# Hansard-T/FHE-Linformer

Measured on AMD Instinct MI355X. Metric: encrypted Linformer-d128 forward ms/sample, lower is better.
Workload: dtype u64

## Files before the change

fhe-linformer_amd/csrc/kernels_elem.hip:

```cpp
#include <hip/hip_runtime.h>
#include <cstdlib>
#include <type_traits>
#include "kernels.h"
#include "kernels_elem.h"

namespace fhelin {
namespace {

typedef u64 u64x2 __attribute__((ext_vector_type(2)));

__device__ __forceinline__ Barrett load_barrett(const DeviceTables& t, int limb) {
    Barrett b;
    b.q = t.moduli[limb];
    b.r0 = t.barrett[2 * limb];
    b.r1 = t.barrett[2 * limb + 1];
    return b;
}

template <int OP>
__global__ __launch_bounds__(256) void ew_binary_kernel(DeviceTables t, u64* out, const u64* a, const u64* b, int b_mod,
                                                        int limb_first, int limb_count) {
    const int v = blockIdx.y;
    const int limb = limb_first + v % limb_count;
    const size_t n2 = (size_t)blockIdx.x * 256 + threadIdx.x;
    const size_t row = ((size_t)1 << t.log_n) >> 1;
    const u64x2 x = reinterpret_cast<const u64x2*>(a)[(size_t)v * row + n2];
    const u64x2 y = reinterpret_cast<const u64x2*>(b)[(size_t)(v % b_mod) * row + n2];
    u64x2 r;
    if (OP == 0) {
        const Barrett br = load_barrett(t, limb);
        r.x = mul_mod(x.x, y.x, br);
        r.y = mul_mod(x.y, y.y, br);
    } else if (OP == 1) {
        const u64 q = t.moduli[limb];
        r.x = add_mod(x.x, y.x, q);
        r.y = add_mod(x.y, y.y, q);
    } else {
        const u64 q = t.moduli[limb];
        r.x = sub_mod(x.x, y.x, q);
        r.y = sub_mod(x.y, y.y, q);
    }
    reinterpret_cast<u64x2*>(out)[(size_t)v * row + n2] = r;
}

template <int OP>
__global__ __launch_bounds__(256) void ew_items_kernel(DeviceTables t, EwItems it, int limb_count) {
    const int item = blockIdx.y / it.vecs, v = blockIdx.y % it.vecs;
    const int limb = v % limb_count;
    const size_t n2 = (size_t)blockIdx.x * 256 + threadIdx.x;
    const size_t row = ((size_t)1 << t.log_n) >> 1;
    const u64x2 x = reinterpret_cast<const u64x2*>(it.a[item])[(size_t)v * row + n2];
    u64x2 r = x;
    if (OP != 4 && (OP != 3 || v < it.b_vecs)) {
        const u64x2 y = reinterpret_cast<const u64x2*>(it.b[item])[(size_t)(v % it.b_vecs) * row + n2];
        if (OP == 0) {
            const Barrett br = load_barrett(t, limb);
            r.x = mul_mod(x.x, y.x, br);
            r.y = mul_mod(x.y, y.y, br);
        } else if (OP == 2) {
            const u64 q = t.moduli[limb];
            r.x = sub_mod(x.x, y.x, q);
            r.y = sub_mod(x.y, y.y, q);
        } else {
            const u64 q = t.moduli[limb];
            r.x = add_mod(x.x, y.x, q);
            r.y = add_mod(x.y, y.y, q);
        }
    }
    reinterpret_cast<u64x2*>(it.out[item])[(size_t)v * row + n2] = r;
}

__global__ __launch_bounds__(256) void ew_dot_kernel(DeviceTables t, u64* out, EwItems it, int limb_count) {
    const int v = blockIdx.y;
    const Barrett br = load_barrett(t, v % limb_count);
    const size_t n2 = (size_t)blockIdx.x * 256 + threadIdx.x;
    const size_t row = ((size_t)1 << t.log_n) >> 1;
    Acc128 ax = {0, 0}, ay = {0, 0};
    for (int i = 0; i < it.n; ++i) {
        const u64x2 x = reinterpret_cast<const u64x2*>(it.a[i])[(size_t)v * row + n2];
        const u64x2 y = reinterpret_cast<const u64x2*>(it.b[i])[(size_t)(v % it.b_vecs) * row + n2];
        acc_mac(ax, x.x, y.x);
        acc_mac(ay, x.y, y.y);
    }
    u64x2 r;
    r.x = barrett_reduce128(ax.lo, ax.hi, br);
    r.y = barrett_reduce128(ay.lo, ay.hi, br);
    reinterpret_cast<u64x2*>(out)[(size_t)v * row + n2] = r;
}

template <int NA>
__global__ __launch_bounds__(256) __attribute__((amdgpu_waves_per_eu(NA <= 8 ? 4 : 3))) void ew_dot_groups_kernel(DeviceTables t, EwDotGroups d) {
    const unsigned nx = gridDim.x, nblk = gridDim.x * gridDim.y;
    unsigned id = blockIdx.y * nx + blockIdx.x;
    if ((nblk & 7) == 0) id = (id & 7) * (nblk >> 3) + (id >> 3);
    const int comp = (int)(id & 1);
    const unsigned rest = id >> 1;
    const int xb = (int)(rest % (unsigned)d.nbatch);
    const int bx = (int)((rest / (unsigned)d.nbatch) % nx), tt = (int)((rest / (unsigned)d.nbatch) / nx);
    const Barrett br = load_barrett(t, tt);
    const size_t n2 = (size_t)bx * 256 + threadIdx.x;
    const size_t row = ((size_t)1 << t.log_n) >> 1;
    const size_t op = (size_t)tt * row + n2, oc = (size_t)(comp * d.ell + tt) * row + n2;
    u64x2 a[NA];
#pragma unroll
    for (int b = 0; b < NA; ++b) a[b] = reinterpret_cast<const u64x2*>(d.a[b] + (size_t)xb * d.a_stride[b])[oc];
    if constexpr (NA <= 8) {
        u64x2 w[NA], wn[NA];
#pragma unroll
        for (int b = 0; b < NA; ++b) w[b] = reinterpret_cast<const u64x2*>(d.p[0][b])[op];
        for (int g = 0; g < d.ng; ++g) {
            const int gn = g + 1 < d.ng ? g + 1 : g;
#pragma unroll
            for (int b = 0; b < NA; ++b) wn[b] = reinterpret_cast<const u64x2*>(d.p[gn][b])[op];
            Acc128 x = {0, 0}, y = {0, 0};
            const u32 m = d.pmask[g];
#pragma unroll
            for (int b = 0; b < NA; ++b)
                if (m >> b & 1u) {
                    acc_mac(x, a[b].x, w[b].x);
                    acc_mac(y, a[b].y, w[b].y);
                }
            u64x2 r;
            r.x = barrett_reduce128(x.lo, x.hi, br);
            r.y = barrett_reduce128(y.lo, y.hi, br);
            reinterpret_cast<u64x2*>(d.out[g] + (size_t)xb * d.out_stride[g])[oc] = r;
#pragma unroll
            for (int b = 0; b < NA; ++b) w[b] = wn[b];
        }
    } else {
        for (int g = 0; g < d.ng; ++g) {
            Acc128 x = {0, 0}, y = {0, 0};
            const u32 m = d.pmask[g];
#pragma unroll
            for (int b0 = 0; b0 < NA; b0 += 8) {
                u64x2 w[8];
#pragma unroll
                for (int b = 0; b < 8; ++b) w[b] = reinterpret_cast<const u64x2*>(d.p[g][b0 + b])[op];
#pragma unroll
                for (int b = 0; b < 8; ++b)
                    if (m >> (b0 + b) & 1u) {
                        acc_mac(x, a[b0 + b].x, w[b].x);
                        acc_mac(y, a[b0 + b].y, w[b].y);
                    }
            }
            u64x2 r;
            r.x = barrett_reduce128(x.lo, x.hi, br);
            r.y = barrett_reduce128(y.lo, y.hi, br);
            reinterpret_cast<u64x2*>(d.out[g] + (size_t)xb * d.out_stride[g])[oc] = r;
        }
    }
}

template <int SH>
__device__ __forceinline__ u64 pack_sh(u64 x) { return (x & ((1ull << SH) - 1)) | ((x >> SH) << 32); }
template <int SH>
__device__ __forceinline__ void acc_flush_sh(const Acc30& a, u64& lo, u64& hi) {
    u64 t = lo + a.s0;
    hi += (t < lo);
    lo = t;
    t = lo + (a.s1 << SH);
    hi += (a.s1 >> (64 - SH)) + (t < lo);
    lo = t;
    t = lo + (a.s2 << (2 * SH));
    hi += (a.s2 >> (64 - 2 * SH)) + (t < lo);
    lo = t;
}

#ifndef WSPLIT
#define WSPLIT 1
#endif
template <int I0, int I1, class F>
__device__ __forceinline__ void static_for(F&& f) {
    if constexpr (I0 < I1) {
        f(std::integral_constant<int, I0>{});
        static_for<I0 + 1, I1>(f);
    }
}

template <int SH>
__device__ __forceinline__ void cyclic_body(const DeviceTables& t, const EwCyclic& d, const Barrett& br, u64 (*ml)[256]) {
    constexpr int P = EwCyclic::PERIOD, G = 2;
    const int tt = blockIdx.y;
    const size_t N = (size_t)1 << t.log_n;
    const size_t n = (size_t)blockIdx.x * 256 + threadIdx.x;
    const size_t oc = (size_t)(blockIdx.z * d.ell + tt) * N + n;
    const u32 bm = (u32)(((size_t)tt * N + n) * 8), bc = (u32)(oc * 8);
    auto ld = [](const u64* p, u32 byte_off) -> u64 { return *reinterpret_cast<const u64*>(reinterpret_cast<const char*>(p) + byte_off); };
    {
        u64 mv[P];
#pragma unroll
        for (int j = 0; j < P; ++j) mv[j] = ld(d.m[j], bm);
#pragma unroll
        for (int j = 0; j < P; ++j) ml[j][threadIdx.x] = pack_sh<SH>(mv[j]);
    }
    __builtin_amdgcn_sched_barrier(0);
    u64 a[P];
#pragma unroll
    for (int i = 0; i < P; ++i) a[i] = ld(d.a[i], bc);
#pragma unroll
    for (int i = 0; i < P; ++i) a[i] = i < d.n ? pack_sh<SH>(a[i]) : 0;
#pragma unroll 1
    for (int k = 0; k < P; k += G) {
        u64 lo[G], hi[G];
        Acc30 x[G];
        static_for<0, G>([&](auto I) __attribute__((always_inline)) {
            lo[decltype(I)::value] = hi[decltype(I)::value] = 0;
            x[decltype(I)::value] = Acc30{0, 0, 0};
        });
        static_for<0, P / 8>([&](auto I0) __attribute__((always_inline)) {
            constexpr int i0 = 8 * decltype(I0)::value;
            static_for<i0, i0 + 8>([&](auto I) __attribute__((always_inline)) {
                constexpr int i = decltype(I)::value;
                const u64 w = ml[(i + k) & (P - 1)][threadIdx.x];
                const u32 w0 = (u32)w, w1 = (u32)(w >> 32);
                static_for<0, G>([&](auto Gi) __attribute__((always_inline)) {
                    constexpr int g = decltype(Gi)::value;
                    constexpr int ii = (i - g) & (P - 1);
                    mac30(x[g], (u32)a[ii], (u32)(a[ii] >> 32), w0, w1);
                });
            });
            __builtin_amdgcn_sched_barrier(0);
            if constexpr (SH == 30) {
                static_for<0, G>([&](auto Gi) __attribute__((always_inline)) {
                    constexpr int g = decltype(Gi)::value;
                    acc_flush_sh<30>(x[g], lo[g], hi[g]);
                    x[g] = Acc30{0, 0, 0};
                    if constexpr (i0 == 8) {
                        lo[g] = barrett_reduce128(lo[g], hi[g], br);
                        hi[g] = 0;
                    }
                });
            }
        });
        static_for<0, G>([&](auto Gi) __attribute__((always_inline)) {
            constexpr int g = decltype(Gi)::value;
            if constexpr (SH != 30) acc_flush_sh<SH>(x[g], lo[g], hi[g]);
            d.out[k + g][oc] = barrett_reduce128(lo[g], hi[g], br);
        });
    }
}

__global__ __launch_bounds__(256, 2) void ew_cyclic_dot_kernel(DeviceTables t, EwCyclic d) {
    __shared__ u64 ml[EwCyclic::PERIOD][256];
    const Barrett br = load_barrett(t, blockIdx.y);
    if ((br.q >> 53) == 0)
        cyclic_body<27>(t, d, br, ml);
    else
        cyclic_body<30>(t, d, br, ml);
}

template <int O0, int SH, int G>
__device__ __forceinline__ void window_segment(const EwWindow& d, const Barrett& br, const u64 (&cur)[EwWindow::W], const u64 (&prv)[EwWindow::W],
                                               const u64 (*ml)[256], size_t oc, u64 (&pre)[G]) {
    constexpr int P = EwWindow::W;
#pragma unroll 1
    for (int oo = 0; oo < 8; oo += G) {
        u64 lo[G], hi[G];
        Acc30 x[G][WSPLIT];
        static_for<0, G>([&](auto I) __attribute__((always_inline)) {
            constexpr int i = decltype(I)::value;
            lo[i] = pre[i];
            hi[i] = 0;
            static_for<0, WSPLIT>([&](auto U) __attribute__((always_inline)) { x[i][decltype(U)::value] = Acc30{0, 0, 0}; });
        });
        if (d.accumulate && O0 + oo + G < P) {
            static_for<0, G>([&](auto I) __attribute__((always_inline)) { pre[decltype(I)::value] = d.out[O0 + oo + G + decltype(I)::value][oc]; });
        }
        static_for<0, P / 8>([&](auto J0) __attribute__((always_inline)) {
            constexpr int j0 = 8 * decltype(J0)::value;
            static_for<j0, j0 + 8>([&](auto J) __attribute__((always_inline)) {
                constexpr int j = decltype(J)::value;
                constexpr int c = O0 - j;
                u64 w;
                if constexpr (c >= 0)
                    w = ml[oo + c][threadIdx.x];
                else if constexpr (c + (8 - G) < 0)
                    w = ml[oo + c + P][threadIdx.x];
                else
                    w = ml[(oo + c) & (P - 1)][threadIdx.x];
                const u32 w0 = (u32)w, w1 = (u32)(w >> 32);
                static_for<0, G>([&](auto I) __attribute__((always_inline)) {
                    constexpr int i = decltype(I)::value;
                    constexpr int jj = (j + i) & (P - 1);
                    constexpr int e = jj - O0 - i;
                    u64 a;
                    if constexpr (jj < O0 || e <= 0)
                        a = cur[jj];
                    else if constexpr (jj >= O0 + 8 || e > 8 - G)
                        a = prv[jj];
                    else
                        a = oo >= e ? cur[jj] : prv[jj];
                    mac30(x[i][j % WSPLIT], (u32)a, (u32)(a >> 32), w0, w1);
                });
            });
            if constexpr (SH == 30) {
                static_for<0, G>([&](auto I) __attribute__((always_inline)) {
                    constexpr int i = decltype(I)::value;
                    static_for<0, WSPLIT>([&](auto U) __attribute__((always_inline)) {
                        acc_flush_sh<30>(x[i][decltype(U)::value], lo[i], hi[i]);
                        x[i][decltype(U)::value] = Acc30{0, 0, 0};
                    });
                    if constexpr (j0 == 8 || j0 == 24) {
                        lo[i] = barrett_reduce128(lo[i], hi[i], br);
                        hi[i] = 0;
                    }
                });
            }
        });
        static_for<0, G>([&](auto I) __attribute__((always_inline)) {
            constexpr int i = decltype(I)::value;
            if constexpr (SH != 30) {
                static_for<0, WSPLIT>([&](auto U) __attribute__((always_inline)) { acc_flush_sh<SH>(x[i][decltype(U)::value], lo[i], hi[i]); });
                lo[i] = barrett_reduce128(lo[i], hi[i], br);
            }
            d.out[O0 + oo + i][oc] = lo[i];
        });
    }
}

template <int SH, int G>
__device__ __forceinline__ void window_body(const DeviceTables& t, const EwWindow& d, const Barrett& br, u64 (*ml)[256]) {
    constexpr int P = EwWindow::W;
    const int tt = blockIdx.y;
    const size_t N = (size_t)1 << t.log_n;
    const size_t n = (size_t)blockIdx.x * 256 + threadIdx.x;
    const size_t om = (size_t)tt * N + n, oc = (size_t)(blockIdx.z * d.ell + tt) * N + n;
    {
        u64 mv[P];
#pragma unroll
        for (int k = 0; k < P; ++k) mv[k] = d.m[k][om];
#pragma unroll
        for (int k = 0; k < P; ++k) ml[k][threadIdx.x] = pack_sh<SH>(mv[k]);
    }
    u64 cur[P], prv[P];
    auto load_cur = [&](int j0) {
#pragma unroll
        for (int j = j0; j < j0 + 8; ++j) cur[j] = d.cur[j][oc];
#pragma unroll
        for (int j = j0; j < j0 + 8; ++j) cur[j] = (d.cur_mask >> j & 1u) ? pack_sh<SH>(cur[j]) : 0;
    };
#pragma unroll
    for (int j = 0; j < P; ++j) prv[j] = d.prev[j][oc];
#pragma unroll
    for (int j = 0; j < P; ++j) prv[j] = (d.prev_mask >> j & 1u) ? pack_sh<SH>(prv[j]) : 0;
    load_cur(0);
    load_cur(8);
    u64 pre[G];
#pragma unroll
    for (int i = 0; i < G; ++i) pre[i] = d.accumulate ? d.out[i][oc] : 0;
    window_segment<0, SH, G>(d, br, cur, prv, ml, oc, pre);
    load_cur(16);
    window_segment<8, SH, G>(d, br, cur, prv, ml, oc, pre);
    load_cur(24);
    window_segment<16, SH, G>(d, br, cur, prv, ml, oc, pre);
    window_segment<24, SH, G>(d, br, cur, prv, ml, oc, pre);
}

template <int G>
__global__ __launch_bounds__(256, 2) void ew_window_dot_kernel(DeviceTables t, EwWindow d) {
    __shared__ u64 ml[EwWindow::W][256];
    const Barrett br = load_barrett(t, blockIdx.y);
    if ((br.q >> 53) == 0)
        window_body<27, G>(t, d, br, ml);
    else
        window_body<30, G>(t, d, br, ml);
}

__global__ __launch_bounds__(256) void ew_muladd_kernel(DeviceTables t, u64* out, const u64* acc, const u64* a, const u64* b,
                                                        int b_mod, int limb_first, int limb_count) {
    const int v = blockIdx.y;
    const int limb = limb_first + v % limb_count;
    const size_t n2 = (size_t)blockIdx.x * 256 + threadIdx.x;
    const size_t row = ((size_t)1 << t.log_n) >> 1;
    const Barrett br = load_barrett(t, limb);
    const u64x2 x = reinterpret_cast<const u64x2*>(a)[(size_t)v * row + n2];
    const u64x2 y = reinterpret_cast<const u64x2*>(b)[(size_t)(v % b_mod) * row + n2];
    const u64x2 c = reinterpret_cast<const u64x2*>(acc)[(size_t)v * row + n2];
    u64x2 r;
    r.x = add_mod(c.x, mul_mod(x.x, y.x, br), br.q);
    r.y = add_mod(c.y, mul_mod(x.y, y.y, br), br.q);
    reinterpret_cast<u64x2*>(out)[(size_t)v * row + n2] = r;
}

__global__ __launch_bounds__(256) void ew_neg_kernel(DeviceTables t, u64* out, const u64* a, int limb_first, int limb_count) {
    const int v = blockIdx.y;
    const u64 q = t.moduli[limb_first + v % limb_count];
    const size_t n2 = (size_t)blockIdx.x * 256 + threadIdx.x;
    const size_t row = ((size_t)1 << t.log_n) >> 1;
    const u64x2 x = reinterpret_cast<const u64x2*>(a)[(size_t)v * row + n2];
    u64x2 r;
    r.x = neg_mod(x.x, q);
    r.y = neg_mod(x.y, q);
    reinterpret_cast<u64x2*>(out)[(size_t)v * row + n2] = r;
}

__global__ __launch_bounds__(256) void ew_scalar_kernel(DeviceTables t, u64* out, const u64* a, ScalarSet sc, int limb_first,
                                                        int limb_count, int in_limbs) {
    const int v = blockIdx.y;
    const int li = v % limb_count;
    const u64 q = t.moduli[limb_first + li];
    const u64 w = sc.v[2 * li], ws = sc.v[2 * li + 1];
    const size_t n2 = (size_t)blockIdx.x * 256 + threadIdx.x;
    const size_t row = ((size_t)1 << t.log_n) >> 1;
    const size_t vin = in_limbs > 0 ? (size_t)(v / limb_count) * in_limbs + li : (size_t)v;
    const u64x2 x = reinterpret_cast<const u64x2*>(a)[vin * row + n2];
    u64x2 r;
    r.x = mul_shoup(x.x, w, ws, q);
    r.y = mul_shoup(x.y, w, ws, q);
    reinterpret_cast<u64x2*>(out)[(size_t)v * row + n2] = r;
}

__global__ __launch_bounds__(256) void ew_scalar_items_kernel(DeviceTables t, EwScalarItems d, u64* __restrict__ out,
                                                              const u64* __restrict__ consts) {
    const int vecs = d.npoly * d.ell;
    const int item = blockIdx.y / vecs, v = blockIdx.y % vecs;
    const int limb = v % d.ell;
    const u64 q = t.moduli[limb];
    const u64* k = consts + ((size_t)item * d.ell + limb) * 2;
    const u64 w = k[0], ws = k[1];
    const size_t n2 = (size_t)blockIdx.x * 256 + threadIdx.x;
    const size_t row = ((size_t)1 << t.log_n) >> 1;
    const size_t vin = (size_t)(v / d.ell) * d.in_limbs[item] + limb;
    const u64x2 x = reinterpret_cast<const u64x2*>(d.a[item])[vin * row + n2];
    u64x2 r;
    r.x = mul_shoup(x.x, w, ws, q);
    r.y = mul_shoup(x.y, w, ws, q);
    reinterpret_cast<u64x2*>(out)[((size_t)item * vecs + v) * row + n2] = r;
}

__global__ __launch_bounds__(256) void ew_scaled_diff_kernel(DeviceTables t, EwScaledDiff d, const u64* __restrict__ consts) {
    const int item = blockIdx.y / d.vecs, v = blockIdx.y % d.vecs;
    const int limb = v % d.ell;
    const u64 q = t.moduli[limb];
    const u64* k = consts + ((size_t)item * d.ell + limb) * 4;
    const u64 a = k[0], as = k[1], c = k[2], cs = k[3];
    const size_t n2 = (size_t)blockIdx.x * 256 + threadIdx.x;
    const size_t row = ((size_t)1 << t.log_n) >> 1;
    const size_t at = (size_t)v * row + n2;
    const u64x2 x = reinterpret_cast<const u64x2*>(d.u[item])[at];
    const u64x2 y = reinterpret_cast<const u64x2*>(d.w[item])[at];
    u64x2 r;
    r.x = sub_mod(mul_shoup(x.x, a, as, q), mul_shoup(y.x, c, cs, q), q);
    r.y = sub_mod(mul_shoup(x.y, a, as, q), mul_shoup(y.y, c, cs, q), q);
    reinterpret_cast<u64x2*>(d.out[item])[at] = r;
}

__global__ __launch_bounds__(256) void ew_addscalar_kernel(DeviceTables t, u64* out, const u64* a, ScalarSet sc, int limb_first,
                                                           int limb_count, int add_vecs) {
    const int v = blockIdx.y;
    const int li = v % limb_count;
    const u64 q = t.moduli[limb_first + li];
    const u64 w = v < add_vecs ? sc.v[2 * li] : 0;
    const size_t n2 = (size_t)blockIdx.x * 256 + threadIdx.x;
    const size_t row = ((size_t)1 << t.log_n) >> 1;
    const u64x2 x = reinterpret_cast<const u64x2*>(a)[(size_t)v * row + n2];
    u64x2 r;
    r.x = add_mod(x.x, w, q);
    r.y = add_mod(x.y, w, q);
    reinterpret_cast<u64x2*>(out)[(size_t)v * row + n2] = r;
}

__global__ __launch_bounds__(256) void ew_lincomb_kernel(DeviceTables t, u64* out, LinComb lc, const u64* __restrict__ scal, int ell,
                                                         int in_limbs) {
    const int v = blockIdx.y;
    const int l = v % ell;
    const Barrett br = load_barrett(t, l);
    const size_t n2 = (size_t)blockIdx.x * 256 + threadIdx.x;
    const size_t row = ((size_t)1 << t.log_n) >> 1;
    const size_t vin = in_limbs > 0 ? (size_t)(v / ell) * in_limbs + l : (size_t)v;
    Acc128 ax = {0, 0}, ay = {0, 0};
    for (int k = 0; k < lc.n; ++k) {
        const u64 sk = scal[(size_t)k * ell + l];
        const u64x2 x = reinterpret_cast<const u64x2*>(lc.a[k])[vin * row + n2];
        acc_mac(ax, x.x, sk);
        acc_mac(ay, x.y, sk);
    }
    const u64 c0 = v < ell ? scal[(size_t)lc.n * ell + l] : 0;
    u64x2 r;
    r.x = add_mod(barrett_reduce128(ax.lo, ax.hi, br), c0, br.q);
    r.y = add_mod(barrett_reduce128(ay.lo, ay.hi, br), c0, br.q);
    reinterpret_cast<u64x2*>(out)[(size_t)v * row + n2] = r;
}

__global__ __launch_bounds__(256) void tensor_kernel(DeviceTables t, u64* d, const u64* a, const u64* b, int ell) {
    const int l = blockIdx.y;
    const Barrett br = load_barrett(t, l);
    const size_t n2 = (size_t)blockIdx.x * 256 + threadIdx.x;
    const size_t row = ((size_t)1 << t.log_n) >> 1;
    const size_t poly = (size_t)ell * row;
    const u64x2* A = reinterpret_cast<const u64x2*>(a);
    const u64x2* B = reinterpret_cast<const u64x2*>(b);
    const u64x2 a0 = A[l * row + n2], a1 = A[poly + l * row + n2];
    const u64x2 b0 = B[l * row + n2], b1 = B[poly + l * row + n2];
    u64x2 d0, d1, d2;
    d0.x = mul_mod(a0.x, b0.x, br);
    d0.y = mul_mod(a0.y, b0.y, br);
    d2.x = mul_mod(a1.x, b1.x, br);
    d2.y = mul_mod(a1.y, b1.y, br);
    d1.x = add_mod(mul_mod(a0.x, b1.x, br), mul_mod(a1.x, b0.x, br), br.q);
    d1.y = add_mod(mul_mod(a0.y, b1.y, br), mul_mod(a1.y, b0.y, br), br.q);
    u64x2* D = reinterpret_cast<u64x2*>(d);
    D[l * row + n2] = d0;
    D[poly + l * row + n2] = d1;
    D[2 * poly + l * row + n2] = d2;
}

__global__ __launch_bounds__(256) void tensor_items_kernel(DeviceTables t, EwItems it, int ell) {
    const int l = blockIdx.y, k = blockIdx.z;
    const Barrett br = load_barrett(t, l);
    const size_t n2 = (size_t)blockIdx.x * 256 + threadIdx.x;
    const size_t row = ((size_t)1 << t.log_n) >> 1;
    const size_t poly = (size_t)ell * row;
    const u64x2* A = reinterpret_cast<const u64x2*>(it.a[k]);
    const u64x2* B = reinterpret_cast<const u64x2*>(it.b[k]);
    const u64x2 a0 = A[l * row + n2], a1 = A[poly + l * row + n2];
    const u64x2 b0 = B[l * row + n2], b1 = B[poly + l * row + n2];
    u64x2 d0, d1, d2;
    d0.x = mul_mod(a0.x, b0.x, br);
    d0.y = mul_mod(a0.y, b0.y, br);
    d2.x = mul_mod(a1.x, b1.x, br);
    d2.y = mul_mod(a1.y, b1.y, br);
    d1.x = add_mod(mul_mod(a0.x, b1.x, br), mul_mod(a1.x, b0.x, br), br.q);
    d1.y = add_mod(mul_mod(a0.y, b1.y, br), mul_mod(a1.y, b0.y, br), br.q);
    u64x2* D = reinterpret_cast<u64x2*>(it.out[k]);
    D[l * row + n2] = d0;
    D[poly + l * row + n2] = d1;
    D[2 * poly + l * row + n2] = d2;
}

__global__ __launch_bounds__(256) void automorph_kernel(int log_n, u64* out, const u64* in, const u32* map) {
    const int v = blockIdx.y;
    const size_t n = (size_t)1 << log_n;
    const size_t j = ((size_t)blockIdx.x * 256 + threadIdx.x) * 2;
    const u32 m0 = map[j], m1 = map[j + 1];
    u64x2 r;
    r.x = in[v * n + m0];
    r.y = in[v * n + m1];
    reinterpret_cast<u64x2*>(out)[(v * n + j) >> 1] = r;
}

__global__ __launch_bounds__(256) void automorph_pack30_kernel(DeviceTables t, u64* out, const u64* in, const u32* map) {
    const int v = blockIdx.y;
    const int limb = v % t.n_limbs;
    const u64 q = t.moduli[limb], R = t.mont[2 * limb], Rs = t.mont[2 * limb + 1];
    const size_t n = (size_t)1 << t.log_n;
    const size_t j = ((size_t)blockIdx.x * 256 + threadIdx.x) * 2;
    const u32 m0 = map[j], m1 = map[j + 1];
    u64x2 r;
    r.x = pack30(mul_shoup(in[v * n + m0], R, Rs, q));
    r.y = pack30(mul_shoup(in[v * n + m1], R, Rs, q));
    reinterpret_cast<u64x2*>(out)[(v * n + j) >> 1] = r;
}

__global__ __launch_bounds__(256) void rescale_lift_kernel(DeviceTables t, u64* lifted, const u64* last, int ell1 ,
                                                           const u64* qlmod_row) {
    const int v = blockIdx.y;
    const int p = v / ell1, tq = v % ell1;
    const Barrett br = load_barrett(t, tq);
    const u64 ql = t.moduli[ell1];
    const u64 half = ql >> 1;
    const u64 qlm = qlmod_row[tq];
    const size_t n2 = (size_t)blockIdx.x * 256 + threadIdx.x;
    const size_t row = ((size_t)1 << t.log_n) >> 1;
    const u64x2 x = reinterpret_cast<const u64x2*>(last)[(size_t)p * row + n2];
    u64x2 r;
    r.x = barrett_reduce128(x.x, 0, br);
    r.y = barrett_reduce128(x.y, 0, br);
    if (x.x > half) r.x = sub_mod(r.x, qlm, br.q);
    if (x.y > half) r.y = sub_mod(r.y, qlm, br.q);
    reinterpret_cast<u64x2*>(lifted)[(size_t)v * row + n2] = r;
}

__global__ __launch_bounds__(256) void wrap_mask_kernel(DeviceTables t, const WrapMaskRow* __restrict__ rows) {
    const WrapMaskRow r = rows[blockIdx.z];
    const int l = blockIdx.y;
    if (l >= r.ell) return;
    const size_t N = (size_t)1 << t.log_n;
    const size_t j = ((size_t)blockIdx.x * 256 + threadIdx.x) * 2;
    const Barrett br = load_barrett(t, l);
    const u64* m = r.mask + (size_t)l * N;
    const u64 m0 = m[r.map[j]], m1 = m[r.map[j + 1]];
#pragma unroll
    for (int p = 0; p < 2; ++p) {
        const u64x2 x = *reinterpret_cast<const u64x2*>(r.src + ((size_t)p * r.src_ell + l) * N + j);
        u64x2 y;
        y.x = mul_mod(x.x, m0, br);
        y.y = mul_mod(x.y, m1, br);
        *reinterpret_cast<u64x2*>(r.dst + ((size_t)p * r.ell + l) * N + j) = y;
    }
}

__global__ __launch_bounds__(256) void modraise_kernel(DeviceTables t, u64* out, const u64* src, int src_limb, int nl) {
    const int v = blockIdx.y;
    const int p = v / nl, tq = v % nl;
    const Barrett br = load_barrett(t, tq);
    const u64 qs = t.moduli[src_limb];
    const u64 half = qs >> 1;
    const u64 qsm = barrett_reduce128(qs, 0, br);
    const size_t n2 = (size_t)blockIdx.x * 256 + threadIdx.x;
    const size_t row = ((size_t)1 << t.log_n) >> 1;
    const u64x2 x = reinterpret_cast<const u64x2*>(src)[(size_t)p * row + n2];
    u64x2 r;
    r.x = barrett_reduce128(x.x, 0, br);
    r.y = barrett_reduce128(x.y, 0, br);
    if (x.x > half) r.x = sub_mod(r.x, qsm, br.q);
    if (x.y > half) r.y = sub_mod(r.y, qsm, br.q);
    reinterpret_cast<u64x2*>(out)[(size_t)v * row + n2] = r;
}

__global__ __launch_bounds__(256) void rescale_finish_kernel(DeviceTables t, u64* out, const u64* c, const u64* lifted, int ell1,
                                                             const u64* qlinv_row) {
    const int v = blockIdx.y;
    const int p = v / ell1, tq = v % ell1;
    const u64 q = t.moduli[tq];
    const u64 w = qlinv_row[2 * tq], ws = qlinv_row[2 * tq + 1];
    const size_t n2 = (size_t)blockIdx.x * 256 + threadIdx.x;
    const size_t row = ((size_t)1 << t.log_n) >> 1;
    const u64x2 x = reinterpret_cast<const u64x2*>(c)[((size_t)p * (ell1 + 1) + tq) * row + n2];
    const u64x2 y = reinterpret_cast<const u64x2*>(lifted)[(size_t)v * row + n2];
    u64x2 r;
    r.x = mul_shoup(sub_mod(x.x, y.x, q), w, ws, q);
    r.y = mul_shoup(sub_mod(x.y, y.y, q), w, ws, q);
    reinterpret_cast<u64x2*>(out)[(size_t)v * row + n2] = r;
}

__global__ __launch_bounds__(256) void reduce_i128_kernel(DeviceTables t, u64* out, const u64* coeffs, int limb_first) {
    const int v = blockIdx.y;
    const Barrett br = load_barrett(t, limb_first + v);
    const size_t n = (size_t)blockIdx.x * 256 + threadIdx.x;
    const size_t N = (size_t)1 << t.log_n;
    u64 lo = coeffs[2 * n], hi = coeffs[2 * n + 1];
    const bool neg = (hi >> 63) != 0;
    if (neg) {
        lo = ~lo + 1;
        hi = ~hi + (lo == 0);
    }
    const u64 h = barrett_reduce128(hi, 0, br);
    u64 r = barrett_reduce128(lo, h, br);
    if (neg) r = neg_mod(r, br.q);
    out[(size_t)v * N + n] = r;
}

inline dim3 grid2(int log_n, int nvec) { return dim3((1u << log_n) / 512, (unsigned)nvec); }

}

void launch_ew_items(const DeviceTables& t, const EwItems& it, int op, int limb_count, hipStream_t s) {
    if (it.n <= 0 || it.vecs <= 0) return;
    const dim3 g = grid2(t.log_n, it.n * it.vecs);
    switch (op) {
        case 0: hipLaunchKernelGGL((ew_items_kernel<0>), g, dim3(256), 0, s, t, it, limb_count); break;
        case 1: hipLaunchKernelGGL((ew_items_kernel<1>), g, dim3(256), 0, s, t, it, limb_count); break;
        case 2: hipLaunchKernelGGL((ew_items_kernel<2>), g, dim3(256), 0, s, t, it, limb_count); break;
        case 4: hipLaunchKernelGGL((ew_items_kernel<4>), g, dim3(256), 0, s, t, it, limb_count); break;
        default: hipLaunchKernelGGL((ew_items_kernel<3>), g, dim3(256), 0, s, t, it, limb_count); break;
    }
}
void launch_ew_dot(const DeviceTables& t, u64* out, const EwItems& it, int limb_count, hipStream_t s) {
    if (it.n <= 0 || it.vecs <= 0) return;
    hipLaunchKernelGGL(ew_dot_kernel, grid2(t.log_n, it.vecs), dim3(256), 0, s, t, out, it, limb_count);
}
void launch_ew_dot_groups(const DeviceTables& t, const EwDotGroups& din, hipStream_t s) {
    if (din.na <= 0 || din.ng <= 0 || din.ell <= 0) return;
    EwDotGroups d = din;
    const int width = d.na <= 8 ? 8 : EwDotGroups::MAX_A;
    const u64* any = d.a[0];
    for (int g = 0; g < d.ng && any == d.a[0]; ++g)
        for (int b = 0; b < d.na; ++b)
            if (d.p[g][b]) {
                any = d.p[g][b];
                break;
            }
    for (int b = d.na; b < width; ++b) {
        d.a[b] = d.a[0];
        d.a_stride[b] = d.a_stride[0];
    }
    for (int g = 0; g < d.ng; ++g) {
        d.pmask[g] = 0;
        for (int b = 0; b < width; ++b) {
            if (b < d.na && d.p[g][b])
                d.pmask[g] |= 1u << b;
            else
                d.p[g][b] = any;
        }
    }
    const int nb = d.nbatch > 0 ? d.nbatch : 1;
    if (d.na <= 8)
        hipLaunchKernelGGL((ew_dot_groups_kernel<8>), grid2(t.log_n, 2 * d.ell * nb), dim3(256), 0, s, t, d);
    else
        hipLaunchKernelGGL((ew_dot_groups_kernel<16>), grid2(t.log_n, 2 * d.ell * nb), dim3(256), 0, s, t, d);
}
void launch_ew_cyclic_dot(const DeviceTables& t, const EwCyclic& din, hipStream_t s) {
    if (din.n <= 0 || din.ell <= 0) return;
    EwCyclic d = din;
    for (int i = d.n; i < EwCyclic::PERIOD; ++i) d.a[i] = d.a[0];
    hipLaunchKernelGGL(ew_cyclic_dot_kernel, dim3((1u << t.log_n) / 256, (unsigned)d.ell, 2), dim3(256), 0, s, t, d);
}
void launch_ew_window_dot(const DeviceTables& t, const EwWindow& d, hipStream_t s) {
    if (d.ell <= 0) return;
    static const int group = [] { const char* e = std::getenv("FHELIN_WINDOW_GROUP"); return e ? std::atoi(e) : 2; }();
    const dim3 g((1u << t.log_n) / 256, (unsigned)d.ell, 2);
    switch (group) {
        case 1: hipLaunchKernelGGL(ew_window_dot_kernel<1>, g, dim3(256), 0, s, t, d); break;
        case 4: hipLaunchKernelGGL(ew_window_dot_kernel<4>, g, dim3(256), 0, s, t, d); break;
        default: hipLaunchKernelGGL(ew_window_dot_kernel<2>, g, dim3(256), 0, s, t, d); break;
    }
}
void launch_ew_mul(const DeviceTables& t, u64* out, const u64* a, const u64* b, int nvec, int b_mod, int limb_first, int limb_count, hipStream_t s) {
    if (nvec <= 0) return;
    hipLaunchKernelGGL((ew_binary_kernel<0>), grid2(t.log_n, nvec), dim3(256), 0, s, t, out, a, b, b_mod, limb_first, limb_count);
}
void launch_ew_add(const DeviceTables& t, u64* out, const u64* a, const u64* b, int nvec, int b_mod, int limb_first, int limb_count, hipStream_t s) {
    if (nvec <= 0) return;
    hipLaunchKernelGGL((ew_binary_kernel<1>), grid2(t.log_n, nvec), dim3(256), 0, s, t, out, a, b, b_mod, limb_first, limb_count);
}
void launch_ew_sub(const DeviceTables& t, u64* out, const u64* a, const u64* b, int nvec, int b_mod, int limb_first, int limb_count, hipStream_t s) {
    if (nvec <= 0) return;
    hipLaunchKernelGGL((ew_binary_kernel<2>), grid2(t.log_n, nvec), dim3(256), 0, s, t, out, a, b, b_mod, limb_first, limb_count);
}
void launch_ew_muladd(const DeviceTables& t, u64* out, const u64* acc, const u64* a, const u64* b, int nvec, int b_mod, int limb_first,
                      int limb_count, hipStream_t s) {
    if (nvec <= 0) return;
    hipLaunchKernelGGL(ew_muladd_kernel, grid2(t.log_n, nvec), dim3(256), 0, s, t, out, acc, a, b, b_mod, limb_first, limb_count);
}
void launch_ew_neg(const DeviceTables& t, u64* out, const u64* a, int nvec, int limb_first, int limb_count, hipStream_t s) {
    if (nvec <= 0) return;
    hipLaunchKernelGGL(ew_neg_kernel, grid2(t.log_n, nvec), dim3(256), 0, s, t, out, a, limb_first, limb_count);
}
void launch_ew_scalar(const DeviceTables& t, u64* out, const u64* a, const ScalarSet& sc, int nvec, int limb_first, int limb_count, hipStream_t s,
                      int in_limbs) {
    if (nvec <= 0) return;
    hipLaunchKernelGGL(ew_scalar_kernel, grid2(t.log_n, nvec), dim3(256), 0, s, t, out, a, sc, limb_first, limb_count, in_limbs);
}
void launch_ew_scalar_items(const DeviceTables& t, const EwScalarItems& d, u64* out, const u64* consts, hipStream_t s) {
    if (d.n <= 0 || d.npoly <= 0 || d.ell <= 0) return;
    hipLaunchKernelGGL(ew_scalar_items_kernel, grid2(t.log_n, d.n * d.npoly * d.ell), dim3(256), 0, s, t, d, out, consts);
}
void launch_ew_scaled_diff(const DeviceTables& t, const EwScaledDiff& d, const u64* consts, hipStream_t s) {
    if (d.n <= 0 || d.vecs <= 0 || d.ell <= 0) return;
    hipLaunchKernelGGL(ew_scaled_diff_kernel, grid2(t.log_n, d.n * d.vecs), dim3(256), 0, s, t, d, consts);
}
void launch_ew_addscalar(const DeviceTables& t, u64* out, const u64* a, const ScalarSet& sc, int nvec, int limb_first, int limb_count, hipStream_t s,
                         int add_vecs) {
    if (nvec <= 0) return;
    hipLaunchKernelGGL(ew_addscalar_kernel, grid2(t.log_n, nvec), dim3(256), 0, s, t, out, a, sc, limb_first, limb_count, add_vecs < 0 ? nvec : add_vecs);
}
void launch_ew_lincomb(const DeviceTables& t, u64* out, const LinComb& lc, const u64* scal, int ell, hipStream_t s, int in_limbs) {
    if (lc.n <= 0 || lc.vecs <= 0) return;
    hipLaunchKernelGGL(ew_lincomb_kernel, grid2(t.log_n, lc.vecs), dim3(256), 0, s, t, out, lc, scal, ell, in_limbs);
}
void launch_tensor(const DeviceTables& t, u64* d, const u64* a, const u64* b, int ell, hipStream_t s) {
    hipLaunchKernelGGL(tensor_kernel, grid2(t.log_n, ell), dim3(256), 0, s, t, d, a, b, ell);
}
void launch_tensor_items(const DeviceTables& t, const EwItems& it, int ell, hipStream_t s) {
    if (it.n <= 0) return;
    hipLaunchKernelGGL(tensor_items_kernel, dim3((1u << t.log_n) / 512, (unsigned)ell, (unsigned)it.n), dim3(256), 0, s, t, it, ell);
}
void launch_automorph(const DeviceTables& t, u64* out, const u64* in, const u32* map, int nvec, hipStream_t s) {
    if (nvec <= 0) return;
    hipLaunchKernelGGL(automorph_kernel, grid2(t.log_n, nvec), dim3(256), 0, s, t.log_n, out, in, map);
}
void launch_automorph_pack30(const DeviceTables& t, u64* out, const u64* in, const u32* map, int nvec, hipStream_t s) {
    if (nvec <= 0) return;
    hipLaunchKernelGGL(automorph_pack30_kernel, grid2(t.log_n, nvec), dim3(256), 0, s, t, out, in, map);
}
void launch_wrap_mask(const DeviceTables& t, const WrapMaskRow* rows, int n_rows, int max_ell, hipStream_t s) {
    if (n_rows < 1 || n_rows > 65535 || max_ell < 1 || max_ell > t.n_limbs) return;
    hipLaunchKernelGGL(wrap_mask_kernel, dim3((1u << t.log_n) / 512, (unsigned)max_ell, (unsigned)n_rows), dim3(256), 0, s, t, rows);
}
void launch_rescale_lift(const DeviceTables& t, u64* lifted, const u64* last, int npoly, int ell, const u64* qlmod_row, hipStream_t s) {
    hipLaunchKernelGGL(rescale_lift_kernel, grid2(t.log_n, npoly * (ell - 1)), dim3(256), 0, s, t, lifted, last, ell - 1, qlmod_row);
}
void launch_rescale_finish(const DeviceTables& t, u64* out, const u64* c, const u64* lifted, int npoly, int ell, const u64* qlinv_row,
                           hipStream_t s) {
    hipLaunchKernelGGL(rescale_finish_kernel, grid2(t.log_n, npoly * (ell - 1)), dim3(256), 0, s, t, out, c, lifted, ell - 1, qlinv_row);
}
void launch_modraise(const DeviceTables& t, u64* out, const u64* src, int npoly, int src_limb, int nl, hipStream_t s) {
    hipLaunchKernelGGL(modraise_kernel, grid2(t.log_n, npoly * nl), dim3(256), 0, s, t, out, src, src_limb, nl);
}
void launch_reduce_i128(const DeviceTables& t, u64* out, const u64* coeffs, int limb_first, int nlimbs, hipStream_t s) {
    hipLaunchKernelGGL(reduce_i128_kernel, dim3((1u << t.log_n) / 256, (unsigned)nlimbs), dim3(256), 0, s, t, out, coeffs, limb_first);
}

}
```

Before: 226.3.

## Add 30-bit split-limb dot-groups kernel with Montgomery path and block swizzle

Adds a new ew_dot_groups kernel that splits each operand into 30-bit halves and accumulates with 32-bit multiply-adds instead of 64-bit 128-bit MACs. When there are at least four groups, operands are pre-scaled into Montgomery form and reduced with REDC rather than Barrett. It also swizzles block IDs across XCDs, double-buffers plaintext loads across groups, and uses 32-bit byte offsets with occupancy hints. It is on by default behind an env switch, and it adds complexity and possible register pressure.

```diff
diff --git a/fhe-linformer_amd/csrc/kernels_elem.hip b/fhe-linformer_amd/csrc/kernels_elem.hip
--- a/fhe-linformer_amd/csrc/kernels_elem.hip
+++ b/fhe-linformer_amd/csrc/kernels_elem.hip
@@ -147,6 +147,116 @@
             r.x = barrett_reduce128(x.lo, x.hi, br);
             r.y = barrett_reduce128(y.lo, y.hi, br);
             reinterpret_cast<u64x2*>(d.out[g] + (size_t)xb * d.out_stride[g])[oc] = r;
+        }
+    }
+}
+
+__device__ __forceinline__ void mac30v(Acc30& a, u32 x0, u32 x1, u32 y0, u32 y1) {
+    a.s0 = mad32(x0, y0, a.s0);
+    a.s1 = mad32(x0, y1, a.s1);
+    a.s1 = mad32(x1, y0, a.s1);
+    a.s2 = mad32(x1, y1, a.s2);
+}
+template <int NA, bool MONT>
+__global__ __launch_bounds__(256) __attribute__((amdgpu_waves_per_eu(NA <= 8 ? 4 : 3))) void ew_dot_groups_split_kernel(DeviceTables t, EwDotGroups d) {
+    const unsigned nx = gridDim.x, nblk = gridDim.x * gridDim.y;
+    unsigned id = blockIdx.y * nx + blockIdx.x;
+    if ((nblk & 7) == 0) id = (id & 7) * (nblk >> 3) + (id >> 3);
+    const int comp = (int)(id & 1);
+    const unsigned rest = id >> 1;
+    const int xb = (int)(rest % (unsigned)d.nbatch);
+    const int bx = (int)((rest / (unsigned)d.nbatch) % nx), tt = (int)((rest / (unsigned)d.nbatch) / nx);
+    const size_t n2 = (size_t)bx * 256 + threadIdx.x;
+    const size_t row = ((size_t)1 << t.log_n) >> 1;
+    const u32 bp = (u32)(((size_t)tt * row + n2) * 16), bc = (u32)(((size_t)(comp * d.ell + tt) * row + n2) * 16);
+    auto ld2 = [](const u64* p, u32 byte_off) -> u64x2 { return *reinterpret_cast<const u64x2*>(reinterpret_cast<const char*>(p) + byte_off); };
+    auto here = [](u32 byte_off) -> u32 {
+        asm volatile("" : "+v"(byte_off));
+        return byte_off;
+    };
+    const u64 q = t.moduli[tt];
+    [[maybe_unused]] const u64 qi = MONT ? t.qinv[tt] : 0;
+    [[maybe_unused]] const Barrett br = MONT ? Barrett{q, 0, 0} : load_barrett(t, tt);
+    u32 ax0[NA], ax1[NA], ay0[NA], ay1[NA];
+    {
+        u64x2 a[NA];
+#pragma unroll
+        for (int b = 0; b < NA; ++b) a[b] = ld2(d.a[b] + (size_t)xb * d.a_stride[b], bc);
+        [[maybe_unused]] const u64 R = t.mont[2 * tt], Rs = t.mont[2 * tt + 1];
+#pragma unroll
+        for (int b = 0; b < NA; ++b) {
+            if constexpr (MONT) {
+                a[b].x = mul_shoup(a[b].x, R, Rs, q);
+                a[b].y = mul_shoup(a[b].y, R, Rs, q);
+            }
+            split30(a[b].x, ax0[b], ax1[b]);
+            split30(a[b].y, ay0[b], ay1[b]);
+            asm volatile("" : "+v"(ax0[b]), "+v"(ax1[b]), "+v"(ay0[b]), "+v"(ay1[b]));
+        }
+    }
+    auto terms = [&](const u64x2 (&w)[8], auto B0, u32 m, u64 (&lo)[2], u64 (&hi)[2]) __attribute__((always_inline)) {
+        constexpr int b0 = decltype(B0)::value;
+        Acc30 x = {0, 0, 0}, y = {0, 0, 0};
+#pragma unroll
+        for (int b = 0; b < 8; ++b)
+            if (m >> (b0 + b) & 1u) {
+                u32 w0, w1;
+                split30(w[b].x, w0, w1);
+                mac30v(x, ax0[b0 + b], ax1[b0 + b], w0, w1);
+                split30(w[b].y, w0, w1);
+                mac30v(y, ay0[b0 + b], ay1[b0 + b], w0, w1);
+            }
+        acc30_flush(x, lo[0], hi[0]);
+        acc30_flush(y, lo[1], hi[1]);
+    };
+    auto finish = [&](int g, const u64 (&lo)[2], const u64 (&hi)[2]) __attribute__((always_inline)) {
+        u64x2 r;
+        if constexpr (MONT) {
+            r.x = redc128(lo[0], hi[0], q, qi);
+            r.y = redc128(lo[1], hi[1], q, qi);
+        } else {
+            r.x = barrett_reduce128(lo[0], hi[0], br);
+            r.y = barrett_reduce128(lo[1], hi[1], br);
+        }
+        const u32 bo = here(bc);
+        *reinterpret_cast<u64x2*>(reinterpret_cast<char*>(d.out[g] + (size_t)xb * d.out_stride[g]) + bo) = r;
+    };
+    auto load8 = [&](u64x2 (&w)[8], int g, int b0) __attribute__((always_inline)) {
+        const u32 o = here(bp);
+#pragma unroll
+        for (int b = 0; b < 8; ++b) w[b] = ld2(d.p[g][b0 + b], o);
+    };
+    if constexpr (NA <= 8) {
+        auto group = [&](int g, const u64x2 (&w)[8]) __attribute__((always_inline)) {
+            u64 lo[2] = {0, 0}, hi[2] = {0, 0};
+            terms(w, std::integral_constant<int, 0>{}, d.pmask[g], lo, hi);
+            finish(g, lo, hi);
+        };
+        u64x2 w0[8], w1[8];
+        load8(w0, 0, 0);
+        int g = 0;
+        for (; g + 1 < d.ng; g += 2) {
+            load8(w1, g + 1, 0);
+            group(g, w0);
+            load8(w0, g + 2 < d.ng ? g + 2 : g + 1, 0);
+            group(g + 1, w1);
+        }
+        if (g < d.ng) group(g, w0);
+    } else {
+        for (int g = 0; g < d.ng; ++g) {
+            u64 lo[2] = {0, 0}, hi[2] = {0, 0};
+            const u32 m = d.pmask[g];
+            {
+                u64x2 w[8];
+                load8(w, g, 0);
+                terms(w, std::integral_constant<int, 0>{}, m, lo, hi);
+            }
+            {
+                u64x2 w[8];
+                load8(w, g, 8);
+                terms(w, std::integral_constant<int, 8>{}, m, lo, hi);
+            }
+            finish(g, lo, hi);
         }
     }
 }
@@ -685,10 +795,25 @@
         }
     }
     const int nb = d.nbatch > 0 ? d.nbatch : 1;
-    if (d.na <= 8)
-        hipLaunchKernelGGL((ew_dot_groups_kernel<8>), grid2(t.log_n, 2 * d.ell * nb), dim3(256), 0, s, t, d);
-    else
-        hipLaunchKernelGGL((ew_dot_groups_kernel<16>), grid2(t.log_n, 2 * d.ell * nb), dim3(256), 0, s, t, d);
+    static const bool split = [] { const char* e = std::getenv("FHELIN_DOT_GROUPS_SPLIT"); return e ? std::atoi(e) != 0 : true; }();
+    const dim3 grid = grid2(t.log_n, 2 * d.ell * nb);
+    const bool wide = d.na > 8;
+    if (!split) {
+        if (!wide)
+            hipLaunchKernelGGL((ew_dot_groups_kernel<8>), grid, dim3(256), 0, s, t, d);
+        else
+            hipLaunchKernelGGL((ew_dot_groups_kernel<16>), grid, dim3(256), 0, s, t, d);
+    } else if (d.ng >= 4) {
+        if (!wide)
+            hipLaunchKernelGGL((ew_dot_groups_split_kernel<8, true>), grid, dim3(256), 0, s, t, d);
+        else
+            hipLaunchKernelGGL((ew_dot_groups_split_kernel<16, true>), grid, dim3(256), 0, s, t, d);
+    } else {
+        if (!wide)
+            hipLaunchKernelGGL((ew_dot_groups_split_kernel<8, false>), grid, dim3(256), 0, s, t, d);
+        else
+            hipLaunchKernelGGL((ew_dot_groups_split_kernel<16, false>), grid, dim3(256), 0, s, t, d);
+    }
 }
 void launch_ew_cyclic_dot(const DeviceTables& t, const EwCyclic& din, hipStream_t s) {
     if (din.n <= 0 || din.ell <= 0) return;
```

Result: no change. 225.2 (median of 5 runs) (-0.5%).
